# GabrieleCocco/CLFaceDetection

Hardware: NVIDIA B200
Metric: frames_per_sec_1080p (higher is better)
Workload: dtype f64

## Files before the change

clfacedetection_b200/csrc/clfd_pack.h:

```cpp
#pragma once
#include "clfd_internal.h"

namespace clfd {

struct PackedCascade {
    DenseParams dense[2];
    int dense_stumps = 0;
    std::vector<TailStump> tail[2];
    std::vector<DenseStage> stage_tab[2];
    int patch_cut = 0;
    DenseParams patch;
    std::vector<TailStump> patch_tail;
    std::vector<DeepStage> deep_stages;
    std::vector<DeepNode> deep_nodes;
    std::vector<int> tree_first_node;
    std::vector<float> alpha;
};

void pack_cascade(const HostCascade &c, PackedCascade &out);
void pack_sc_level(const HostCascade &c, double factor, int pitch, ScLevel &L, ScNode *out);
bool pack_sc_dense(const HostCascade &c, double scale, DenseParams &P, std::vector<TailStump> &tail,
                   std::vector<DenseStage> &stage_tab);
const char *get_error();

int dense_tile_stride(int win_w, int ystep);
int dense_tile_half(int win_w, int ystep);
int dense_tile_rows(int win_h, int ystep, int tile_h);
int dense_tile_cols(int win_w, int ystep);

}
```

clfacedetection_b200/csrc/haar_pack.cpp:

```cpp
#include <algorithm>
#include <cfloat>
#include <cmath>
#include <cstdarg>
#include <cstdio>
#include <cstdlib>
#include <cstring>

#include "clfd_pack.h"

namespace clfd {

static thread_local char g_error[1024] = "";

void set_error(const char *fmt, ...) {
    va_list ap;
    va_start(ap, fmt);
    vsnprintf(g_error, sizeof g_error, fmt, ap);
    va_end(ap);
}
const char *get_error() { return g_error; }

#define FMT_FAIL(...) do { set_error(__VA_ARGS__); return CLFD_ERR_FORMAT; } while (0)

int build_hidden(HostCascade &c) {
// ... 302 lines not shown
                const int n = c.tr_first_node[t] + j;
                const HostNode &nd = c.nodes[n];
                any3 |= c.hid_nrects[n] == 3;
                for (int k = 0; k < c.hid_nrects[n]; k++) {
                    int dx[4], dy[4];
                    corner_coords(nd, k, dx, dy);
                    for (int q = 0; q < 4; q++) ts.off[k * 4 + q] = tile_offset(dy[q], dx[q]) + (nd.tilted ? (uint32_t)tilt_base : 0u);
                    ts.w[k] = c.hid_weight[(size_t)n * 3 + k];
                }
                ts.thr = nd.threshold;
                ts.a0 = nd.left <= 0 ? c.alpha[a + (-nd.left)] : 0.f;
                ts.a1 = nd.right <= 0 ? c.alpha[a + (-nd.right)] : 0.f;
                ts.meta = (uint32_t)j | ((nd.left > 0 ? (uint32_t)nd.left : kNodeLeaf) << 8) |
                          ((nd.right > 0 ? (uint32_t)nd.right : kNodeLeaf) << 16);
                amax = fmax(amax, fmax(fabs((double)ts.a0), fabs((double)ts.a1)));
            }
            abs_sum += amax;
        }
        ds.first = 0; ds.count = (uint16_t)(c.st_ntrees[i] * P.npt);
        ds.thr = c.hid_thr[i];
        ds.flags = ((!c.is_tree && c.is_stump_based && c.two_rects[i]) ? 1u : 0u) | (any3 ? 2u : 0u) |
                   (c.order_free[i] ? 4u : 0u);
        const double er = (double)(c.st_ntrees[i] * P.npt) * ldexp(1.0, -23) * abs_sum;
        ds.sum_eps = std::isfinite(er) ? (float)(er * 1.0000002) + FLT_MIN : INFINITY;
        ds.sum_eps += 1.0001e-5f * std::fabs(ds.thr);
        if (walk_tree) {
            const uint32_t pass = c.st_child[i] >= 0 ? (uint32_t)pos[c.st_child[i]] : kRouteAccept;
            int p = i;
            while (p >= 0 && c.st_next[p] < 0) p = c.st_parent[p];
            const uint32_t fail = p >= 0 ? (uint32_t)pos[c.st_next[p]] : kRouteReject;
            ds.flags |= ((uint32_t)i << 8) | (pass << 16) | (fail << 24);
            stage_tab[e] = ds;
        }
        if (e < elig) P.stage[e] = ds;
    }
    const bool share_corners = !getenv("CLFD_NO_SHARED_CORNERS");
    int ns = 0, nstump = 0;
    while (ns < elig && nstump + c.st_ntrees[ns] * P.npt <= kMaxDenseStumps) {
        P.stage[ns].first = (uint16_t)nstump;
        std::vector<DenseStump> six, rest;
        for (int t = c.st_first_tree[ns] * P.npt; t < c.st_first_tree[ns + 1] * P.npt; t++) {
            DenseStump st = tail[t];
            bool shared = false;
            if (share_corners && P.npt == 1 && c.hid_nrects[c.tr_first_node[t]] == 2) {
                const uint32_t *A = st.off, *B = st.off + 4;
                static const int pairs[4][2] = {{0, 2}, {3, 1}, {0, 1}, {3, 2}};
                for (const auto &pr : pairs) {
                    const int pl = pr[0], mi = pr[1];
                    if (A[pl] != B[pl] || A[mi] != B[mi]) continue;
                    const int opl = pl == 0 ? 3 : 0, omi = mi == 1 ? 2 : 1;
                    const uint32_t o[6] = {A[pl], A[mi], A[opl], A[omi], B[opl], B[omi]};
                    for (int q = 0; q < 12; q++) st.off[q] = q < 6 ? o[q] : 0;
                    shared = true;
                    break;
                }
            }
            (shared ? six : rest).push_back(st);
        }
        P.stage[ns].n_shared = (uint32_t)six.size();
        for (const auto &st : six) P.stump[nstump++] = st;
        for (const auto &st : rest) P.stump[nstump++] = st;
        ns++;
    }
    P.n_stages = ns;
    {
        static_assert(sizeof(TailStump) == 80, "five 16-byte chunks per record");
        struct Chunk { uint32_t v[4]; };
        std::vector<TailStump> blocked;
        const Chunk *src = reinterpret_cast<const Chunk *>(tail.data());
        int at = 0;
        for (int e = 0; e < E; e++) {
            const int count = c.st_ntrees[order[e]] * P.npt;
            const size_t first = blocked.size();
            blocked.resize(first + (size_t)((count + 31) / 32) * 32);
            Chunk *blk = reinterpret_cast<Chunk *>(blocked.data() + first);
            for (int j = 0; j < count; j++)
                for (int q = 0; q < 5; q++) blk[(size_t)(j >> 5) * 160 + q * 32 + (j & 31)] = src[(size_t)(at + j) * 5 + q];
            if (e < elig) P.stage[e].tail_first = (uint32_t)first;
            if (walk_tree) stage_tab[e].tail_first = (uint32_t)first;
            at += count;
        }
        tail.swap(blocked);
    }
    P.pool_min = 0;
    if (const char *e = getenv("CLFD_POOL_MIN")) P.pool_min = std::max(0, atoi(e));
    P.track_abs = 0;
    for (float v : c.alpha)
        if (std::fabs(v) > 64.f) P.track_abs = 1;
    if (getenv("CLFD_NO_TRACK_ABS")) P.track_abs = 0;
    int nf = 3;
    if (const char *e = getenv("CLFD_N_FIXED")) nf = atoi(e);
    P.n_fixed = nf < 0 ? 0 : (nf > ns ? ns : nf);
}

void pack_cascade(const HostCascade &c, PackedCascade &out) {
    const int S = c.n_stages(), T = c.n_trees(), N = c.n_nodes();
    out.deep_stages.resize(S);
    out.deep_nodes.resize(N);
    out.tree_first_node = c.tr_first_node;
    out.alpha = c.alpha;
    for (int i = 0; i < S; i++) {
        DeepStage &s = out.deep_stages[i];
        memset(&s, 0, sizeof s);
        s.first_tree = c.st_first_tree[i];
        s.ntrees = c.st_ntrees[i];
        s.thr = c.hid_thr[i];
        bool stumps = true;
        for (int t = s.first_tree; t < s.first_tree + s.ntrees; t++) stumps &= c.tr_nnodes[t] == 1;
        const bool dbl = !c.is_tree && c.is_stump_based && c.two_rects[i];
        s.flags = (dbl ? 1 : 0) | (c.order_free[i] ? 2 : 0) | (stumps ? 4 : 0);
        s.parent = c.st_parent[i]; s.next = c.st_next[i]; s.child = c.st_child[i];
    }
    for (int n = 0; n < N; n++) {
        DeepNode &d = out.deep_nodes[n];
        memset(&d, 0, sizeof d);
        const HostNode &nd = c.nodes[n];
        for (int k = 0; k < c.hid_nrects[n]; k++) {
            int dx[4], dy[4];
            corner_coords(nd, k, dx, dy);
            for (int q = 0; q < 4; q++) { d.dx[k * 4 + q] = (uint8_t)dx[q]; d.dy[k * 4 + q] = (uint8_t)dy[q]; }
            d.w[k] = c.hid_weight[(size_t)n * 3 + k];
        }
        d.thr = nd.threshold;
        d.left = nd.left; d.right = nd.right;
        d.flags = (nd.tilted ? 1 : 0) | (c.hid_nrects[n] << 8);
    }

    for (int yi = 0; yi < 2; yi++) pack_dense_one(c, yi + 1, out.dense[yi], out.tail[yi], out.stage_tab[yi], out.dense_stumps);
    out.patch_cut = 0;
    const DenseParams &D = out.dense[0];
    const bool finishes = D.tail_stages == S && D.exec_stages == S && out.dense[1].tail_stages == S;
    if (finishes && !c.has_tilted && !c.is_tree && c.is_stump_based && D.npt == 1 && !D.track_abs && !out.dense[1].track_abs && S >= 8) {
        int cut = 0;
        if (const char *e = getenv("CLFD_PATCH_CUT")) cut = atoi(e);
        if (cut > 0 && cut < S) {
            cut = std::max(cut, std::max(D.n_fixed, out.dense[1].n_fixed));
            std::vector<DenseStage> no_tab;
            int n_stumps = 0;
            pack_dense_one(c, 1, out.patch, out.patch_tail, no_tab, n_stumps, (c.win_w + 1) | 1);
            if (out.patch.tail_stages == S && cut < S) {
                out.patch_cut = cut;
                for (int yi = 0; yi < 2; yi++) out.dense[yi].cut_stages = cut;
            }
        }
    }
}

bool pack_sc_dense(const HostCascade &c, double scale, DenseParams &P, std::vector<TailStump> &tail,
                   std::vector<DenseStage> &stage_tab) {
    HostCascade s = c;
    const int ex = cv_round_d(scale), ey = ex;
    const int ew = cv_round_d((c.win_w - 2) * scale), eh = cv_round_d((c.win_h - 2) * scale);
    const double weight_scale = 1. / (ew * eh);
    int ext_w = std::max(cv_round_d(c.win_w * scale), ex + ew), ext_h = std::max(cv_round_d(c.win_h * scale), ey + eh);
    for (int n = 0; n < c.n_nodes(); n++) {
        const HostNode &nd = c.nodes[n];
        HostNode &d = s.nodes[n];
        const int nr = c.hid_nrects[n];
        double sum0 = 0, area0 = 0;
        const double correction_ratio = weight_scale * (!nd.tilted ? 1 : 0.5);
        for (int k = 0; k < nr; k++) {
            d.rect[k][0] = cv_round_d(nd.rect[k][0] * scale); d.rect[k][2] = cv_round_d(nd.rect[k][2] * scale);
            d.rect[k][1] = cv_round_d(nd.rect[k][1] * scale); d.rect[k][3] = cv_round_d(nd.rect[k][3] * scale);
            int dx[4], dy[4];
            corner_coords(d, k, dx, dy);
            for (int q = 0; q < 4; q++) {
                if (dx[q] < 0 || dy[q] < 0) return false;
                ext_w = std::max(ext_w, dx[q]); ext_h = std::max(ext_h, dy[q]);
            }
            float &w = s.hid_weight[(size_t)n * 3 + k];
            w = (float)(nd.weight[k] * correction_ratio);
            if (k == 0) area0 = d.rect[k][2] * d.rect[k][3];
            else sum0 += w * d.rect[k][2] * d.rect[k][3];
// ... 13 lines not shown
```

clfacedetection_b200/csrc/kernels_clod.cu:

```cuda
#include <algorithm>
#include <cstdint>

#include "clfd_pack.h"
#include "kernels.h"

namespace clfd {

typedef unsigned long long ull;

__device__ __forceinline__ uint32_t smem_u32(const void *p) { return (uint32_t)__cvta_generic_to_shared(p); }

__device__ __forceinline__ void mbar_init(uint64_t *bar, uint32_t count) {
    asm volatile("mbarrier.init.shared::cta.b64 [%0], %1;" ::"r"(smem_u32(bar)), "r"(count));
    asm volatile("fence.mbarrier_init.release.cluster;" ::: "memory");
}
__device__ __forceinline__ void mbar_expect_tx(uint64_t *bar, uint32_t bytes) {
    asm volatile("mbarrier.arrive.expect_tx.shared::cta.b64 _, [%0], %1;" ::"r"(smem_u32(bar)), "r"(bytes) : "memory");
}
__device__ __forceinline__ void mbar_wait(uint64_t *bar, uint32_t parity) {
    asm volatile(
        "{\n"
        ".reg .pred P1;\n"
        "LAB_WAIT:\n"
        "mbarrier.try_wait.parity.shared::cta.b64 P1, [%0], %1;\n"
        "@P1 bra DONE;\n"
        "bra LAB_WAIT;\n"
        "DONE:\n"
        "}" ::"r"(smem_u32(bar)), "r"(parity) : "memory");
}
__device__ __forceinline__ void tma_bulk_g2s(void *dst_smem, const void *src_gmem, uint32_t bytes, uint64_t *bar) {
    asm volatile("cp.async.bulk.shared::cluster.global.mbarrier::complete_tx::bytes [%0], [%1], %2, [%3];"
                 ::"r"(smem_u32(dst_smem)), "l"(src_gmem), "r"(bytes), "r"(smem_u32(bar)) : "memory");
}

__device__ __forceinline__ double window_sigma(int s4, ull q4, double inv_area) {
    const double mean = __dmul_rn((double)s4, inv_area);
    const double v = __dsub_rn(__dmul_rn((double)q4, inv_area), __dmul_rn(mean, mean));
    return v >= 0. ? sqrt(v) : 1.;
}

__device__ __forceinline__ ull sq_rect(const ull *sq, bool sq32, size_t at, int g0, int g1, int g2, int g3) {
    if (sq32) {
        const uint32_t *q = reinterpret_cast<const uint32_t *>(sq) + at;
        return (ull)(uint32_t)(__ldg(q + g0) - __ldg(q + g1) - __ldg(q + g2) + __ldg(q + g3));
    }
    const ull *q = sq + at;
    return __ldg(q + g0) - __ldg(q + g1) - __ldg(q + g2) + __ldg(q + g3);
}

__device__ __forceinline__ void emit_rect(const CascadeArgs &a, const CasLevel &CL, int frame, int px, int py) {
    if (!a.rects) return;
    const ull slot = atomicAdd(a.counters + 0, 1ull);
    if (slot < a.rect_cap) {
        DevRect r;
        r.x = __double2int_rn(__dmul_rn((double)px, CL.factor));
        r.y = __double2int_rn(__dmul_rn((double)py, CL.factor));
        r.w = CL.win_w; r.h = CL.win_h; r.frame = a.frame_base + frame; r.cascade = a.cascade_index;
        a.rects[slot] = r;
    } else {
        atomicAdd(a.counters + 2, 1ull);
    }
}

__device__ __forceinline__ int lds32(uint32_t addr) {
    int v;
    asm volatile("ld.shared.s32 %0, [%1];" : "=r"(v) : "r"(addr));
    return v;
}
template <int IMM>
__device__ __forceinline__ int lds32i(uint32_t addr) {
    int v;
    asm volatile("ld.shared.s32 %0, [%1+%2];" : "=r"(v) : "r"(addr), "n"(IMM));
    return v;
}

#ifdef CLFD_POOLED_STAGES
constexpr bool kPooledStages = true;
#else
constexpr bool kPooledStages = false;
#endif
struct DenseSmemPlan {
    size_t tile, sgf, list, pool, ctl, bar, act, tgt, total;
};
constexpr int kCtlCount = 0, kCtlCountB = 32, kCtlCountC = 64, kCtlInts = 96;
__host__ __device__ inline DenseSmemPlan dense_smem_plan(const DenseParams &P) {
    DenseSmemPlan p;
    const size_t rows = (size_t)(P.tile_h - 1) * P.ystep + P.win_h + 1, windows = (size_t)kTileW * P.tile_h;
    p.tile = 0;
    p.sgf = (rows * P.tile_stride * 4 + 127) & ~(size_t)127;
    if (P.tilted_tile) p.sgf *= 2;
    p.list = p.sgf + windows * sizeof(float);
    p.pool = p.list + windows * sizeof(uint16_t);
    p.ctl = p.pool + (P.pool_min > 0 ? windows * sizeof(uint16_t) : 0);
    p.bar = p.ctl + kCtlInts * sizeof(int);
    p.act = p.tgt = p.total = p.bar + 16;
    if (P.exec_stages > P.tail_stages) {
        p.tgt = p.act + windows * sizeof(uint16_t);
        p.total = p.tgt + windows;
    }
    return p;
}
#ifdef CLFD_TILES_COUNT_TU
constexpr bool kTilesCount = true;
#else
constexpr bool kTilesCount = false;
size_t dense_smem_bytes(const DenseParams &P) { return dense_smem_plan(P).total; }
#endif

struct DenseCtx {
    uint32_t tile;
    const ull *gsq;
    size_t sq_at;
    bool sq32;
    int16_t *codes;
    int sq_pitch;
    int row_mul;
    int ystep, S, half;
    int tx, wy_tile, nx;
    int code_mul;
};

__device__ __forceinline__ uint32_t dense_base(const DenseCtx &c, int wid) {
    return c.tile + (uint32_t)((wid / kTileW) * c.row_mul + (wid & (kTileW - 1)) * 4);
}
__device__ __forceinline__ uint32_t dense_tile_off(const DenseCtx &c, int y, int x) {
    return 4u * (uint32_t)(c.ystep == 1 ? y * c.S + x : y * c.S + (x & 1) * c.half + (x >> 1));
}
__device__ __forceinline__ void dense_write_code(const DenseCtx &c, int wid, int code) {
    const int wx = wid & (kTileW - 1), wy = wid / kTileW;
    c.codes[(size_t)(c.wy_tile + wy) * c.nx + c.tx * kTileW + wx] = (int16_t)code;
}

__device__ __forceinline__ double dense_sigma(const DenseParams &P, const DenseCtx &c, int wid) {
    const int wx = wid & (kTileW - 1), wy = wid / kTileW;
    const int ex = P.eq_x, ey = P.eq_y, eq_w = P.eq_w, eq_h = P.eq_h;
    const uint32_t base = dense_base(c, wid);
    const int s4 = lds32(base + dense_tile_off(c, ey, ex)) - lds32(base + dense_tile_off(c, ey, ex + eq_w)) -
                   lds32(base + dense_tile_off(c, ey + eq_h, ex)) + lds32(base + dense_tile_off(c, ey + eq_h, ex + eq_w));
    const int g0 = ey * c.sq_pitch + ex, g1 = g0 + eq_w, g2 = (ey + eq_h) * c.sq_pitch + ex, g3 = g2 + eq_w;
    const ull q4 = sq_rect(c.gsq, c.sq32, c.sq_at + (size_t)(wy * c.ystep) * c.sq_pitch + wx * c.ystep, g0, g1, g2, g3);
    return window_sigma(s4, q4, P.inv_area);
}
__device__ __forceinline__ double dense_sigma_flat(const DenseParams &P, const DenseCtx &c, int wid, bool &eq_flat) {
    const int wx = wid & (kTileW - 1), wy = wid / kTileW;
    const int ex = P.eq_x, ey = P.eq_y, eq_w = P.eq_w, eq_h = P.eq_h;
    const uint32_t base = dense_base(c, wid);
    const int s4 = lds32(base + dense_tile_off(c, ey, ex)) - lds32(base + dense_tile_off(c, ey, ex + eq_w)) -
                   lds32(base + dense_tile_off(c, ey + eq_h, ex)) + lds32(base + dense_tile_off(c, ey + eq_h, ex + eq_w));
    const int g0 = ey * c.sq_pitch + ex, g1 = g0 + eq_w, g2 = (ey + eq_h) * c.sq_pitch + ex, g3 = g2 + eq_w;
    const ull q4 = sq_rect(c.gsq, c.sq32, c.sq_at + (size_t)(wy * c.ystep) * c.sq_pitch + wx * c.ystep, g0, g1, g2, g3);
    eq_flat = q4 * (ull)(eq_w * eq_h) == (ull)((long long)s4 * s4);
    return window_sigma(s4, q4, P.inv_area);
}

constexpr int kNotFlat = -0x8000;
static __device__ __noinline__ int flat_window_code(const DenseParams &P, const DenseCtx &c, int wid) {
    const uint32_t base = dense_base(c, wid);
    const int W = P.win_w, H = P.win_h;
    const uint32_t S4 = (uint32_t)(lds32(base + dense_tile_off(c, 0, 0)) - lds32(base + dense_tile_off(c, 0, W)) -
                                   lds32(base + dense_tile_off(c, H, 0)) + lds32(base + dense_tile_off(c, H, W)));
    const ull Q4 = sq_rect(c.gsq, c.sq32, c.sq_at + (size_t)((wid / kTileW) * c.ystep) * c.sq_pitch + (wid & (kTileW - 1)) * c.ystep,
                           0, W, H * c.sq_pitch, H * c.sq_pitch + W);
    const uint32_t A = (uint32_t)(W * H);
    if (Q4 * (ull)A != (ull)S4 * (ull)S4) return kNotFlat;
    return (int)__ldg(P.flat_code + S4 / A);
}

struct StumpRegs {
    uint32_t o[12];
    float w0, w1, w2, thr, a0, a1;
    uint32_t meta;
};
__device__ __forceinline__ StumpRegs stump_from_param(const DenseStump &q) {
    StumpRegs r;
#pragma unroll
    for (int i = 0; i < 12; i++) r.o[i] = q.off[i];
    r.w0 = q.w[0]; r.w1 = q.w[1]; r.w2 = q.w[2]; r.thr = q.thr; r.a0 = q.a0; r.a1 = q.a1; r.meta = q.meta;
    return r;
}
__device__ __forceinline__ StumpRegs stump_from_global(const uint4 *__restrict__ rec, int j, bool any3) {
    rec += (j >> 5) * 160 + (j & 31);
    const uint4 q0 = __ldg(rec), q1 = __ldg(rec + 32), q3 = __ldg(rec + 96), q4 = __ldg(rec + 128);
    uint4 q2 = make_uint4(0u, 0u, 0u, 0u);
    if (any3) q2 = __ldg(rec + 64);
    StumpRegs r;
    r.o[0] = q0.x; r.o[1] = q0.y; r.o[2] = q0.z; r.o[3] = q0.w;
    r.o[4] = q1.x; r.o[5] = q1.y; r.o[6] = q1.z; r.o[7] = q1.w;
    r.o[8] = q2.x; r.o[9] = q2.y; r.o[10] = q2.z; r.o[11] = q2.w;
    r.w0 = __uint_as_float(q3.x); r.w1 = __uint_as_float(q3.y); r.w2 = __uint_as_float(q3.z); r.thr = __uint_as_float(q3.w);
// ... 79 lines not shown
    const float d = __fmaf_rn(-q.thr, sg[KK], s32);
    if (NODES) {
        const bool on = at[KK] == (q.meta & 255u);
        near[KK] = near[KK] || (on && fabsf(d) <= m);
        S[KK] = __fadd_rn(S[KK], on ? (d >= 0.f ? q.a1 : q.a0) : 0.f);
        at[KK] = on ? ((d >= 0.f ? q.meta >> 16 : q.meta >> 8) & 255u) : at[KK];
    } else {
        near[KK] = near[KK] || (fabsf(d) <= m);
        const float sel = d >= 0.f ? q.a1 : q.a0;
        S[KK] = __fadd_rn(S[KK], sel);
        if (TRACK) Sa[KK] = __fadd_rn(Sa[KK], fabsf(sel));
    }
}

template <int K, bool FIXED, int ROWSTEP, bool SHARED, bool NODES, bool TRACK>
__device__ __forceinline__ void stump_filter(const StumpRegs &q, bool dbl, bool any3, float eps, const uint32_t (&base)[K],
                                             const float (&sg)[K], float (&S)[K], bool (&near)[K], uint32_t (&at)[K], float (&Sa)[K]) {
    static_assert(K >= 1 && K <= 4, "1..4 windows per thread");
    const bool three = !SHARED && any3 && q.o[11] != 0u;
    uint32_t c[12];
    if (FIXED) {
#pragma unroll
        for (int i = 0; i < (SHARED ? 6 : 12); i++) c[i] = base[0] + q.o[i];
    }
    if (NODES && (q.meta & 255u) == 0u) {
#pragma unroll
        for (int k = 0; k < K; k++) at[k] = 0u;
    }
    stump_filter_window<0, K, FIXED, ROWSTEP, SHARED, NODES, TRACK>(q, dbl, three, eps, c, base, sg, S, near, at, Sa);
    if (K > 1) stump_filter_window<(K > 1 ? 1 : 0), K, FIXED, ROWSTEP, SHARED, NODES, TRACK>(q, dbl, three, eps, c, base, sg, S, near, at, Sa);
    if (K > 2) stump_filter_window<(K > 2 ? 2 : 0), K, FIXED, ROWSTEP, SHARED, NODES, TRACK>(q, dbl, three, eps, c, base, sg, S, near, at, Sa);
    if (K > 3) stump_filter_window<(K > 3 ? 3 : 0), K, FIXED, ROWSTEP, SHARED, NODES, TRACK>(q, dbl, three, eps, c, base, sg, S, near, at, Sa);
}

template <int K, bool FIXED, int ROWSTEP, bool NODES, bool TRACK>
__device__ __forceinline__ void stage_filter(const DenseParams &P, const DenseStage &st, bool resident, int grp, int G,
                                             const uint32_t (&base)[K], const float (&sg)[K], float (&S)[K], bool (&near)[K],
                                             float (&Sa)[K]) {
    uint32_t at[K];
#pragma unroll
    for (int k = 0; k < K; k++) at[k] = 0u;
    const int count = st.count;
    const uint32_t flags = st.flags;
    const bool dbl = flags & 1u, any3 = flags & 2u;
    const float eps = P.filter_eps;
    if (resident && G == 1) {
        const int first = st.first, n6 = (int)st.n_shared;
#pragma unroll 1
        for (int j = 0; j < n6; j++) stump_filter<K, FIXED, ROWSTEP, true, false, TRACK>(stump_from_param(P.stump[first + j]), dbl, false, eps, base, sg, S, near, at, Sa);
#pragma unroll 1
        for (int j = n6; j < count; j++) stump_filter<K, FIXED, ROWSTEP, false, NODES, TRACK>(stump_from_param(P.stump[first + j]), dbl, any3, eps, base, sg, S, near, at, Sa);
    } else {
        const uint4 *__restrict__ rec = reinterpret_cast<const uint4 *>(P.tail + st.tail_first);
        if (NODES) {
            const int npt = P.npt;
#pragma unroll 1
            for (int j = grp * npt; j < count; j += G * npt)
#pragma unroll 1
                for (int i = 0; i < npt; i++)
                    stump_filter<K, FIXED, ROWSTEP, false, true, TRACK>(stump_from_global(rec, j + i, any3), dbl, any3, eps, base, sg, S, near, at, Sa);
        } else {
#pragma unroll 1
            for (int j = grp; j < count; j += G) stump_filter<K, FIXED, ROWSTEP, false, false, TRACK>(stump_from_global(rec, j, any3), dbl, any3, eps, base, sg, S, near, at, Sa);
        }
    }
}

template <bool NODES, bool COUNT, bool TRACK>
__device__ __forceinline__ bool stage_verdict(const DenseParams &P, const DenseCtx &c, const DenseStage &st, float sthr, float seps,
                                              int wid, float S, bool near, float Sa) {
    if (TRACK && !P.force_exact)
        seps = __fadd_ru(__fmul_ru(__fmul_ru((float)st.count, 1.1920930e-7f), Sa), __fadd_ru(__fmul_ru(1.0001e-5f, fabsf(sthr)), 1.2e-38f));
    if (near || !(fabsf(__fadd_rn(S, -sthr)) > seps)) {
        const int r = dense_stage_exact<NODES>(P, c, st.tail_first, st.count, st.flags & 1u, st.thr, wid);
        if (COUNT) {
            atomicAdd(&s_dense_exact, 1u);
            if (r & 2) atomicAdd(&s_dense_near, 1u);
        }
        return r & 1;
    }
    return S >= sthr;
}

template <int ROWSTEP_T, bool TREE, bool NODES, int TILE_H, bool COUNT, bool TRACK>
__device__ __forceinline__ void cascade_tiles_body(const DenseParams &P, const CascadeArgs &a, const int tile0, unsigned char *smem_raw) {
    const DenseSmemPlan plan = dense_smem_plan(P);
    unsigned char *tile = smem_raw + plan.tile;
    float *sgf = reinterpret_cast<float *>(smem_raw + plan.sgf);
    uint16_t *list = reinterpret_cast<uint16_t *>(smem_raw + plan.list);
    int *ctl = reinterpret_cast<int *>(smem_raw + plan.ctl);
    uint64_t *bar = reinterpret_cast<uint64_t *>(smem_raw + plan.bar);

    const int tid = threadIdx.x, lane = tid & 31, warp = tid >> 5;
    const int frame = blockIdx.y;
    const int tile_id = tile0 + blockIdx.x;

    int cl = 0;
    {
        int lo = 0, hi = a.n_cas_levels - 1;
        while (lo < hi) {
            const int mid = (lo + hi + 1) >> 1;
            if (__ldg(&a.cas_levels[mid].tile_base) <= tile_id) lo = mid; else hi = mid - 1;
        }
        cl = lo;
    }
    const CasLevel CL = a.cas_levels[cl];
    const PyrLevel L = a.levels[CL.pyr_level];
    const int local = tile_id - CL.tile_base;
    const int tx = local % CL.tiles_x, ty = local / CL.tiles_x;
    const int ystep = P.ystep;
    constexpr int kTileWindows = kTileW * TILE_H, kDenseSlots = kTileWindows / kDenseThreads;
    constexpr int kDenseChunk = kDenseSlots % 4 == 0 ? 4 : 3;
    static_assert(kDenseSlots % kDenseChunk == 0 && kDenseSlots <= 8, "tile height: 12, 16, 24 or 32 window rows");
    const int px0 = tx * kTileW * ystep, py0 = ty * TILE_H * ystep;
    const int n_wx = min(kTileW, CL.nx - tx * kTileW), n_wy = min(TILE_H, CL.ny - ty * TILE_H);
    const int rows = min((TILE_H - 1) * ystep + P.win_h + 1, L.h + 1 - py0);
    const int cols = ((kTileW - 1) * ystep + P.win_w + 1 + 3) & ~3;
    const int S = P.tile_stride;

    const size_t frame_off = (size_t)frame * a.sum_frame_stride + L.sum_off;
    const int32_t *__restrict__ gsum = a.sum + frame_off + (size_t)py0 * L.sum_pitch + px0;

    for (int i = tid; i < kCtlInts; i += kDenseThreads) ctl[i] = 0;
    if (tid == 0) s_dense_exact = s_dense_near = s_dense_done = 0u;
#ifdef CLFD_TILE_TIMING
    const long long t_start = clock64();
    if (tid == 0) s_dense_t_busy = s_dense_t_p1 = 0u;
#endif
    const int n_tiles_smem = P.tilted_tile ? 2 : 1;
    const size_t tile2_off = ((size_t)((TILE_H - 1) * ystep + P.win_h + 1) * S * 4 + 127) & ~(size_t)127;
    const int32_t *__restrict__ gtil = a.tilted ? a.tilted + frame_off + (size_t)py0 * L.sum_pitch + px0 : gsum;
    if (ystep == 1) {
        if (tid == 0) mbar_init(bar, 1);
        __syncthreads();
        if (tid == 0) mbar_expect_tx(bar, (uint32_t)(rows * cols * 4 * n_tiles_smem));
        for (int r = tid; r < rows * n_tiles_smem; r += kDenseThreads) {
            const int t2 = r >= rows, rr = t2 ? r - rows : r;
            tma_bulk_g2s(tile + (t2 ? tile2_off : 0) + (size_t)rr * S * 4, (t2 ? gtil : gsum) + (size_t)rr * L.sum_pitch,
                         (uint32_t)(cols * 4), bar);
        }
        mbar_wait(bar, 0);
    } else {
        const bool di = a.sum_di != 0;
        const int half = P.tile_half;
        if (di) {
            if (tid == 0) mbar_init(bar, 1);
            __syncthreads();
            const uint32_t hb = (uint32_t)half * 4u;
            if (tid == 0) mbar_expect_tx(bar, (uint32_t)rows * 2u * hb);
            const int32_t *__restrict__ gdi = a.sum + frame_off + (size_t)py0 * L.sum_pitch + (px0 >> 1);
            for (int r = tid; r < rows * 2; r += kDenseThreads) {
                const int odd = r >= rows, rr = odd ? r - rows : r;
                tma_bulk_g2s(tile + (size_t)rr * S * 4 + (odd ? hb : 0u), gdi + (size_t)rr * L.sum_pitch + (odd ? (L.sum_pitch >> 1) : 0), hb, bar);
            }
        }
        const int c4 = cols >> 2, total = rows * c4;
        for (int i = (di ? total : 0) + tid; i < total * n_tiles_smem; i += kDenseThreads) {
            const int t2 = i >= total, ii = t2 ? i - total : i;
            const int r = ii / c4, cq = ii - r * c4;
            const int4 v = __ldg(reinterpret_cast<const int4 *>((t2 ? gtil : gsum) + (size_t)r * L.sum_pitch) + cq);
            int *row = reinterpret_cast<int *>(tile + (t2 ? tile2_off : 0)) + r * S;
            *reinterpret_cast<int2 *>(row + 2 * cq) = make_int2(v.x, v.z);
            *reinterpret_cast<int2 *>(row + half + 2 * cq) = make_int2(v.y, v.w);
        }
        __syncthreads();
        if (di) mbar_wait(bar, 0);
    }

    DenseCtx c;
    c.tile = smem_u32(tile); c.gsq = a.sq; c.sq_at = frame_off + (size_t)py0 * L.sum_pitch + px0; c.sq32 = a.sq32 != 0;
    c.codes = a.codes ? a.codes + (size_t)frame * a.windows_per_frame + CL.win_base : nullptr;
    c.sq_pitch = L.sum_pitch;
    c.row_mul = ystep * S * 4;
    c.ystep = ystep; c.S = S; c.half = P.tile_half;
    c.tx = tx; c.wy_tile = ty * TILE_H; c.nx = CL.nx;
    c.code_mul = P.is_tree ? 2 : 1;
    const float inf = __int_as_float(0x7f800000);

    constexpr int kRowsPerSlot = kDenseThreads / kTileW;
    const int wx = tid & (kTileW - 1), wy0 = tid / kTileW;
    uint32_t alive = 0;
#pragma unroll
    for (int k = 0; k < kDenseSlots; k++) {
        const int wy = wy0 + k * kRowsPerSlot;
        const int wid = wy * kTileW + wx;
        if (wx < n_wx && wy < n_wy) {
            bool eq_flat, live = true;
            sgf[wid] = (float)dense_sigma_flat(P, c, wid, eq_flat);
            if (!COUNT && eq_flat && P.flat_code) {
                const int code = flat_window_code(P, c, wid);
                if (code != kNotFlat) {
                    live = false;
                    if (P.is_tree ? (code & 1) : (code == P.total_stages)) emit_rect(a, CL, frame, px0 + wx * ystep, py0 + wy * ystep);
                }
            }
            if (live) alive |= 1u << k;
        } else {
            sgf[wid] = 1.0f;
        }
    }
    int s = 0;
    for (; s < P.n_fixed; s++) {
        const float sthr = P.stage[s].thr, seps = P.force_exact ? inf : P.stage[s].sum_eps;
#pragma unroll 1
        for (int k0 = 0; k0 < kDenseSlots; k0 += kDenseChunk) {
            const uint32_t m4 = (alive >> k0) & ((1u << kDenseChunk) - 1u);
            if (!__any_sync(0xffffffffu, m4 != 0)) continue;
            uint32_t base[kDenseChunk];
            float sg[kDenseChunk];
            float Ssum[kDenseChunk];
            bool near[kDenseChunk];
#pragma unroll
            for (int k = 0; k < kDenseChunk; k++) {
                const int wy = wy0 + (k0 + k) * kRowsPerSlot;
                base[k] = c.tile + (uint32_t)(wy * c.row_mul + wx * 4);
                sg[k] = sgf[wy * kTileW + wx];
                Ssum[k] = 0.f;
                near[k] = false;
            }
            float Sabs[kDenseChunk];
#pragma unroll
            for (int k = 0; k < kDenseChunk; k++) Sabs[k] = 0.f;
            if (ROWSTEP_T) stage_filter<kDenseChunk, true, ROWSTEP_T, NODES, TRACK>(P, P.stage[s], true, 0, 1, base, sg, Ssum, near, Sabs);
            else stage_filter<kDenseChunk, false, 0, NODES, TRACK>(P, P.stage[s], true, 0, 1, base, sg, Ssum, near, Sabs);
#pragma unroll
            for (int k = 0; k < kDenseChunk; k++) {
                if (!((m4 >> k) & 1u)) continue;
                const int wid = (wy0 + (k0 + k) * kRowsPerSlot) * kTileW + wx;
                if (!stage_verdict<NODES, COUNT, TRACK>(P, c, P.stage[s], sthr, seps, wid, Ssum[k], near[k], Sabs[k])) {
                    alive &= ~(1u << (k0 + k));
                    if (c.codes) dense_write_code(c, wid, s * c.code_mul);
                }
            }
        }
    }

    constexpr int kClassCap = kTileWindows / 32;
    constexpr int kSeg = kTileWindows / kDenseWarps;
    int n_alive;
    uint16_t *cur;
    if (kPooledStages && P.pool_min > 0) {
        uint16_t *cl_in = list, *cl_out = reinterpret_cast<uint16_t *>(smem_raw + plan.pool);
        int *cnt_in = ctl + kCtlCount, *cnt_out = ctl + kCtlCountB, *cnt_zero = ctl + kCtlCountC;
        {
            const int na = __popc(alive);
            if (na) {
                const int cq = (wx + 8 * wy0) & 31;
                int at = atomicAdd(cnt_in + cq, na);
    #pragma unroll
                for (int k = 0; k < kDenseSlots; k++)
                    if ((alive >> k) & 1u) cl_in[cq * kClassCap + at++] = (uint16_t)((wy0 + k * kRowsPerSlot) * kTileW + wx);
            }
        }
        __syncthreads();
            for (;; s++) {
            const int h = cnt_in[lane];
            int incl = h, hmax = h;
    #pragma unroll
            for (int d = 1; d < 32; d <<= 1) {
                const int v = __shfl_up_sync(0xffffffffu, incl, d);
                if (lane >= d) incl += v;
                hmax = max(hmax, __shfl_xor_sync(0xffffffffu, hmax, d));
            }
            const int excl = incl - h, tot = __shfl_sync(0xffffffffu, incl, 31);
            if (tot == 0) return;
            n_alive = tot;
            if (!(P.pool_min > 0 && tot > P.pool_min && s < P.tail_stages)) {
                for (int r = warp; r < h; r += kDenseWarps) {
                    const int i = excl + r;
                    const int w = i % kDenseWarps, p = i / kDenseWarps;
                    const int nw = (tot - w + kDenseWarps - 1) / kDenseWarps, Rw = (nw + 31) >> 5;
                    const int col = p / Rw, row = p - col * Rw;
                    cl_out[w * kSeg + row * 32 + col] = cl_in[lane * kClassCap + r];
                }
                __syncthreads();
                break;
            }
            int R = (tot + 31) >> 5;
            {
                int best = 0x7fffffff;
                for (int r = R; r <= hmax; r++) {
                    int e = max(h - r, 0);
    #pragma unroll
                    for (int d = 16; d > 0; d >>= 1) e += __shfl_xor_sync(0xffffffffu, e, d);
                    const int cost = r * 9 + 5 * min(r, e);
                    if (cost < best) { best = cost; R = r; }
                }
            }
            const int q = (R + kDenseWarps - 1) / kDenseWarps;
            const int r_begin = warp * q, r_end = min(R, r_begin + q);
            if (tid < 32) cnt_zero[tid] = 0;
            const float sthr = P.stage[s].thr, seps = P.force_exact ? inf : P.stage[s].sum_eps;
            auto fetch = [&](int r, bool &valid) -> int {
                const int i = r + lane * R;
                valid = i < tot;
                int cc = 0;
    #pragma unroll
                for (int step = 16; step > 0; step >>= 1) {
                    const int e_t = __shfl_sync(0xffffffffu, excl, (cc + step) & 31);
                    if (e_t <= i) cc += step;
                }
                const int e_c = __shfl_sync(0xffffffffu, excl, cc);
                return valid ? (int)cl_in[cc * kClassCap + (i - e_c)] : 0;
            };
            auto keep_pool = [&](bool valid, int wid, float Ssum, bool near, float Sabs) {
                const bool pass = valid && stage_verdict<NODES, COUNT, TRACK>(P, c, P.stage[s], sthr, seps, wid, Ssum, near, Sabs);
                if (pass) {
                    const int cq = (wid + 8 * (wid / kTileW)) & 31;
                    cl_out[cq * kClassCap + atomicAdd(cnt_out + cq, 1)] = (uint16_t)wid;
                }
                if (valid && !pass && c.codes) dense_write_code(c, wid, s * c.code_mul);
            };
            for (int r = r_begin; r < r_end; r += 2) {
                bool v0, v1 = false;
                const int wid0 = fetch(r, v0);
                if (r + 1 < r_end) {
                    const int wid1 = fetch(r + 1, v1);
                    const uint32_t base[2] = {dense_base(c, wid0), dense_base(c, wid1)};
                    const float sg[2] = {sgf[wid0], sgf[wid1]};
                    float Ssum[2] = {0.f, 0.f};
                    bool near[2] = {false, false};
                    float Sabs[2] = {0.f, 0.f};
                    stage_filter<2, false, 0, NODES, TRACK>(P, P.stage[s], s < P.n_stages, 0, 1, base, sg, Ssum, near, Sabs);
                    keep_pool(v0, wid0, Ssum[0], near[0], Sabs[0]);
                    keep_pool(v1, wid1, Ssum[1], near[1], Sabs[1]);
                } else {
                    const uint32_t base[1] = {dense_base(c, wid0)};
                    const float sg[1] = {sgf[wid0]};
                    float Ssum[1] = {0.f};
                    bool near[1] = {false};
                    float Sabs[1] = {0.f};
                    stage_filter<1, false, 0, NODES, TRACK>(P, P.stage[s], s < P.n_stages, 0, 1, base, sg, Ssum, near, Sabs);
                    keep_pool(v0, wid0, Ssum[0], near[0], Sabs[0]);
                }
            }
            __syncthreads();
            uint16_t *tl = cl_in; cl_in = cl_out; cl_out = tl;
            int *tc = cnt_in; cnt_in = cnt_out; cnt_out = cnt_zero; cnt_zero = tc;
        }

        cur = cl_out + warp * kSeg;
    } else {
        const int na = __popc(alive), cq = (wx + 8 * wy0) & 31;
        int at = na ? atomicAdd(ctl + kCtlCount + cq, na) : 0;
        __syncthreads();
        const int h = ctl[kCtlCount + lane];
        int incl = h;
#pragma unroll
        for (int d = 1; d < 32; d <<= 1) {
            const int v = __shfl_up_sync(0xffffffffu, incl, d);
            if (lane >= d) incl += v;
        }
        n_alive = __shfl_sync(0xffffffffu, incl, 31);
        if (n_alive == 0) return;
        at += __shfl_sync(0xffffffffu, incl - h, cq);
#pragma unroll
        for (int k = 0; k < kDenseSlots; k++) {
            if ((alive >> k) & 1u) {
                const int i = at++;
                const int w = i % kDenseWarps, p = i / kDenseWarps;
                const int nw = (n_alive - w + kDenseWarps - 1) / kDenseWarps, Rw = (nw + 31) >> 5;
                const int col = p / Rw, row = p - col * Rw;
                list[w * kSeg + row * 32 + col] = (uint16_t)((wy0 + k * kRowsPerSlot) * kTileW + wx);
            }
        }
        __syncthreads();
        cur = list + warp * kSeg;
    }

#ifdef CLFD_TILE_TIMING
    if (lane == 0) atomicAdd(&s_dense_t_p1, (unsigned int)(clock64() - t_start));
#endif
    int n = (n_alive - warp + kDenseWarps - 1) / kDenseWarps;
    bool dealt = true;
    for (; s < P.cut_stages && n > 0; s++) {
        const float sthr = P.stage[s].thr, seps = P.force_exact ? inf : P.stage[s].sum_eps;
        int n_next = 0;
        auto keep = [&](bool valid, int wid, float Ssum, bool near, float Sabs) {
            const bool pass = valid && stage_verdict<NODES, COUNT, TRACK>(P, c, P.stage[s], sthr, seps, wid, Ssum, near, Sabs);
            const unsigned m = __ballot_sync(0xffffffffu, pass);
            if (pass) cur[n_next + __popc(m & ((1u << lane) - 1u))] = (uint16_t)wid;
            n_next += __popc(m);
            if (valid && !pass && c.codes) dense_write_code(c, wid, s * c.code_mul);
        };
        if (n > P.g1_min) {
            const int R = (n + 31) >> 5;
            for (int r = 0; r < R; r += 2) {
                const int c0 = dealt ? (n - r + R - 1) / R : min(32, n - 32 * r);
                if (r + 1 < R) {
                    const int c1 = dealt ? (n - r - 1 + R - 1) / R : min(32, n - 32 * (r + 1));
                    const bool v0 = lane < c0, v1 = lane < c1;
                    const int wid0 = cur[32 * r + (v0 ? lane : 0)], wid1 = cur[32 * r + 32 + (v1 ? lane : 0)];
                    __syncwarp();
                    const uint32_t base[2] = {dense_base(c, wid0), dense_base(c, wid1)};
                    const float sg[2] = {sgf[wid0], sgf[wid1]};
                    float Ssum[2] = {0.f, 0.f};
                    bool near[2] = {false, false};
                    float Sabs[2] = {0.f, 0.f};
                    stage_filter<2, false, 0, NODES, TRACK>(P, P.stage[s], s < P.n_stages, 0, 1, base, sg, Ssum, near, Sabs);
                    keep(v0, wid0, Ssum[0], near[0], Sabs[0]);
                    keep(v1, wid1, Ssum[1], near[1], Sabs[1]);
                } else {
                    const bool v0 = lane < c0;
                    const int wid0 = cur[32 * r + (v0 ? lane : 0)];
                    __syncwarp();
                    const uint32_t base[1] = {dense_base(c, wid0)};
                    const float sg[1] = {sgf[wid0]};
                    float Ssum[1] = {0.f};
                    bool near[1] = {false};
                    float Sabs[1] = {0.f};
                    stage_filter<1, false, 0, NODES, TRACK>(P, P.stage[s], s < P.n_stages, 0, 1, base, sg, Ssum, near, Sabs);
                    keep(v0, wid0, Ssum[0], near[0], Sabs[0]);
                }
            }
        } else {
            int lw = 4;
            while (lw > 0 && (1 << (lw - 1)) >= n) lw--;
            const int slot = lane & ((1 << lw) - 1), grp = lane >> lw, G = 32 >> lw;
            const bool valid = slot < n;
            const int wid0 = cur[valid ? slot : 0];
            __syncwarp();
            const uint32_t base[1] = {dense_base(c, wid0)};
            const float sg[1] = {sgf[wid0]};
            float Ssum[1] = {0.f};
            bool near[1] = {false};
            float Sabs[1] = {0.f};
            if (valid) stage_filter<1, false, 0, NODES, TRACK>(P, P.stage[s], s < P.n_stages, grp, G, base, sg, Ssum, near, Sabs);
            float acc = Ssum[0], acc_abs = Sabs[0];
            unsigned nr = near[0];
            for (int d = 1 << lw; d < 32; d <<= 1) {
                acc = __fadd_rn(acc, __shfl_xor_sync(0xffffffffu, acc, d));
                if (TRACK) acc_abs = __fadd_rn(acc_abs, __shfl_xor_sync(0xffffffffu, acc_abs, d));
                nr |= __shfl_xor_sync(0xffffffffu, nr, d);
            }
            keep(lane < n, wid0, acc, nr != 0, acc_abs);
        }
        __syncwarp();
        n = n_next;
        dealt = false;
    }
    if (TREE) {
        if (n == 0) return;
        uint16_t *act = reinterpret_cast<uint16_t *>(smem_raw + plan.act) + warp * kSeg;
        unsigned char *tgt = smem_raw + plan.tgt;
        const int e0 = s;
        for (int e = e0; e < P.exec_stages && n > 0; e++) {
            int n_wait = 0, n_act = 0;
            const int R = (n + 31) >> 5;
            for (int r = 0; r < R; r++) {
                const int c0 = dealt ? (n - r + R - 1) / R : min(32, n - 32 * r);
                const bool v = lane < c0;
// ... 658 lines not shown
```

Baseline: 2856.

## Enable pooled cross-warp stage evaluation with dynamic row claiming by default

Turns the previously compile-time-disabled pooled stage path into a default runtime path for stump cascades when it does not reduce CTAs per SM. Surviving windows are pooled across the whole CTA, and warps claim row pairs dynamically through a shared atomic counter. This replaces static per-warp segments so early stages stay load-balanced as windows die out. It also simplifies the row-count choice to a heuristic and lowers the default fixed-stage count when pooling is on. The cost is extra shared memory, additional __syncthreads and atomics per stage.

```diff
diff --git a/clfacedetection_b200/csrc/clfd_pack.h b/clfacedetection_b200/csrc/clfd_pack.h
--- a/clfacedetection_b200/csrc/clfd_pack.h
+++ b/clfacedetection_b200/csrc/clfd_pack.h
@@ -27,5 +27,6 @@
 int dense_tile_half(int win_w, int ystep);
 int dense_tile_rows(int win_h, int ystep, int tile_h);
 int dense_tile_cols(int win_w, int ystep);
+bool dense_pooled(const DenseParams &P);
 
 }
diff --git a/clfacedetection_b200/csrc/haar_pack.cpp b/clfacedetection_b200/csrc/haar_pack.cpp
--- a/clfacedetection_b200/csrc/haar_pack.cpp
+++ b/clfacedetection_b200/csrc/haar_pack.cpp
@@ -408,13 +408,15 @@
         }
         tail.swap(blocked);
     }
-    P.pool_min = 0;
+    constexpr int kPoolMin = 256;
+    P.pool_min = !c.is_tree && P.npt == 1 && patch_stride == 0 ? kPoolMin : 0;
     if (const char *e = getenv("CLFD_POOL_MIN")) P.pool_min = std::max(0, atoi(e));
+    if (!dense_pooled(P)) P.pool_min = 0;
     P.track_abs = 0;
     for (float v : c.alpha)
         if (std::fabs(v) > 64.f) P.track_abs = 1;
     if (getenv("CLFD_NO_TRACK_ABS")) P.track_abs = 0;
-    int nf = 3;
+    int nf = P.pool_min > 0 ? 2 : 3;
     if (const char *e = getenv("CLFD_N_FIXED")) nf = atoi(e);
     P.n_fixed = nf < 0 ? 0 : (nf > ns ? ns : nf);
 }
diff --git a/clfacedetection_b200/csrc/kernels_clod.cu b/clfacedetection_b200/csrc/kernels_clod.cu
--- a/clfacedetection_b200/csrc/kernels_clod.cu
+++ b/clfacedetection_b200/csrc/kernels_clod.cu
@@ -74,27 +74,32 @@
     return v;
 }
 
-#ifdef CLFD_POOLED_STAGES
-constexpr bool kPooledStages = true;
-#else
-constexpr bool kPooledStages = false;
-#endif
 struct DenseSmemPlan {
     size_t tile, sgf, list, pool, ctl, bar, act, tgt, total;
+    bool pooled;
 };
-constexpr int kCtlCount = 0, kCtlCountB = 32, kCtlCountC = 64, kCtlInts = 96;
+constexpr int kCtlClaim = 64, kCtlInts = 96;
+constexpr size_t kSmemPerSm = 228 * 1024, kSmemPerCta = 1024 + 64;
+constexpr int kDenseCtasPerSm = 4;
+__host__ __device__ inline int dense_ctas_per_sm(size_t bytes) {
+    const int n = (int)(kSmemPerSm / (bytes + kSmemPerCta));
+    return n < kDenseCtasPerSm ? n : kDenseCtasPerSm;
+}
 __host__ __device__ inline DenseSmemPlan dense_smem_plan(const DenseParams &P) {
     DenseSmemPlan p;
     const size_t rows = (size_t)(P.tile_h - 1) * P.ystep + P.win_h + 1, windows = (size_t)kTileW * P.tile_h;
+    const size_t act = P.exec_stages > P.tail_stages ? windows * sizeof(uint16_t) + windows : 0;
     p.tile = 0;
     p.sgf = (rows * P.tile_stride * 4 + 127) & ~(size_t)127;
     if (P.tilted_tile) p.sgf *= 2;
     p.list = p.sgf + windows * sizeof(float);
     p.pool = p.list + windows * sizeof(uint16_t);
-    p.ctl = p.pool + (P.pool_min > 0 ? windows * sizeof(uint16_t) : 0);
+    const size_t fixed = p.pool + kCtlInts * sizeof(int) + 16 + act;
+    p.pooled = P.pool_min > 0 && dense_ctas_per_sm(fixed + windows * sizeof(uint16_t)) == dense_ctas_per_sm(fixed);
+    p.ctl = p.pool + (p.pooled ? windows * sizeof(uint16_t) : 0);
     p.bar = p.ctl + kCtlInts * sizeof(int);
     p.act = p.tgt = p.total = p.bar + 16;
-    if (P.exec_stages > P.tail_stages) {
+    if (act) {
         p.tgt = p.act + windows * sizeof(uint16_t);
         p.total = p.tgt + windows;
     }
@@ -105,6 +110,7 @@
 #else
 constexpr bool kTilesCount = false;
 size_t dense_smem_bytes(const DenseParams &P) { return dense_smem_plan(P).total; }
+bool dense_pooled(const DenseParams &P) { return dense_smem_plan(P).pooled; }
 #endif
 
 struct DenseCtx {
@@ -350,6 +356,24 @@
     return S >= sthr;
 }
 
+__device__ __forceinline__ void class_prefix(int h, int &excl, int &tot, int &hmax) {
+    const int lane = threadIdx.x & 31;
+    int incl = h;
+    hmax = h;
+#pragma unroll
+    for (int d = 1; d < 32; d <<= 1) {
+        const int v = __shfl_up_sync(0xffffffffu, incl, d);
+        if (lane >= d) incl += v;
+        hmax = max(hmax, __shfl_xor_sync(0xffffffffu, hmax, d));
+    }
+    excl = incl - h;
+    tot = __shfl_sync(0xffffffffu, incl, 31);
+}
+__device__ __forceinline__ int pooled_rows(int n, int hmax) {
+    const int r0 = (n + 31) >> 5;
+    return min(hmax, r0 + ((r0 + 3) >> 2));
+}
+
 template <int ROWSTEP_T, bool TREE, bool NODES, int TILE_H, bool COUNT, bool TRACK>
 __device__ __forceinline__ void cascade_tiles_body(const DenseParams &P, const CascadeArgs &a, const int tile0, unsigned char *smem_raw) {
     const DenseSmemPlan plan = dense_smem_plan(P);
@@ -505,93 +529,56 @@
 
     constexpr int kClassCap = kTileWindows / 32;
     constexpr int kSeg = kTileWindows / kDenseWarps;
-    int n_alive;
-    uint16_t *cur;
-    if (kPooledStages && P.pool_min > 0) {
-        uint16_t *cl_in = list, *cl_out = reinterpret_cast<uint16_t *>(smem_raw + plan.pool);
-        int *cnt_in = ctl + kCtlCount, *cnt_out = ctl + kCtlCountB, *cnt_zero = ctl + kCtlCountC;
-        {
-            const int na = __popc(alive);
-            if (na) {
-                const int cq = (wx + 8 * wy0) & 31;
-                int at = atomicAdd(cnt_in + cq, na);
-    #pragma unroll
-                for (int k = 0; k < kDenseSlots; k++)
-                    if ((alive >> k) & 1u) cl_in[cq * kClassCap + at++] = (uint16_t)((wy0 + k * kRowsPerSlot) * kTileW + wx);
+    const int na = __popc(alive), cq = (wx + 8 * wy0) & 31;
+    int *const cnt0 = ctl + 32 * ((s & 1) ^ 1);
+    int at = na ? atomicAdd(cnt0 + cq, na) : 0;
+    __syncthreads();
+    int h = cnt0[lane], excl, n_alive, hmax;
+    class_prefix(h, excl, n_alive, hmax);
+    if (n_alive == 0) return;
+    at += __shfl_sync(0xffffffffu, excl, cq);
+    if (plan.pooled && n_alive > P.pool_min && s < P.cut_stages) {
+        uint16_t *const cls = list + kTileWindows;
+        int R = pooled_rows(n_alive, hmax);
+#pragma unroll
+        for (int k = 0; k < kDenseSlots; k++) {
+            if ((alive >> k) & 1u) {
+                const int i = at++;
+                list[(i % R) * 32 + i / R] = (uint16_t)((wy0 + k * kRowsPerSlot) * kTileW + wx);
             }
         }
         __syncthreads();
-            for (;; s++) {
-            const int h = cnt_in[lane];
-            int incl = h, hmax = h;
-    #pragma unroll
-            for (int d = 1; d < 32; d <<= 1) {
-                const int v = __shfl_up_sync(0xffffffffu, incl, d);
-                if (lane >= d) incl += v;
-                hmax = max(hmax, __shfl_xor_sync(0xffffffffu, hmax, d));
-            }
-            const int excl = incl - h, tot = __shfl_sync(0xffffffffu, incl, 31);
-            if (tot == 0) return;
-            n_alive = tot;
-            if (!(P.pool_min > 0 && tot > P.pool_min && s < P.tail_stages)) {
-                for (int r = warp; r < h; r += kDenseWarps) {
-                    const int i = excl + r;
-                    const int w = i % kDenseWarps, p = i / kDenseWarps;
-                    const int nw = (tot - w + kDenseWarps - 1) / kDenseWarps, Rw = (nw + 31) >> 5;
-                    const int col = p / Rw, row = p - col * Rw;
-                    cl_out[w * kSeg + row * 32 + col] = cl_in[lane * kClassCap + r];
-                }
-                __syncthreads();
-                break;
-            }
-            int R = (tot + 31) >> 5;
-            {
-                int best = 0x7fffffff;
-                for (int r = R; r <= hmax; r++) {
-                    int e = max(h - r, 0);
-    #pragma unroll
-                    for (int d = 16; d > 0; d >>= 1) e += __shfl_xor_sync(0xffffffffu, e, d);
-                    const int cost = r * 9 + 5 * min(r, e);
-                    if (cost < best) { best = cost; R = r; }
-                }
-            }
-            const int q = (R + kDenseWarps - 1) / kDenseWarps;
-            const int r_begin = warp * q, r_end = min(R, r_begin + q);
-            if (tid < 32) cnt_zero[tid] = 0;
+        for (;;) {
+            int *const cnt = ctl + 32 * (s & 1);
+            if (tid < 32) ctl[32 * ((s & 1) ^ 1) + tid] = 0;
+            const int lim = n_alive - lane * R;
             const float sthr = P.stage[s].thr, seps = P.force_exact ? inf : P.stage[s].sum_eps;
-            auto fetch = [&](int r, bool &valid) -> int {
-                const int i = r + lane * R;
-                valid = i < tot;
-                int cc = 0;
-    #pragma unroll
-                for (int step = 16; step > 0; step >>= 1) {
-                    const int e_t = __shfl_sync(0xffffffffu, excl, (cc + step) & 31);
-                    if (e_t <= i) cc += step;
-                }
-                const int e_c = __shfl_sync(0xffffffffu, excl, cc);
-                return valid ? (int)cl_in[cc * kClassCap + (i - e_c)] : 0;
-            };
-            auto keep_pool = [&](bool valid, int wid, float Ssum, bool near, float Sabs) {
+            auto keep = [&](bool valid, int wid, float Ssum, bool near, float Sabs) {
                 const bool pass = valid && stage_verdict<NODES, COUNT, TRACK>(P, c, P.stage[s], sthr, seps, wid, Ssum, near, Sabs);
                 if (pass) {
-                    const int cq = (wid + 8 * (wid / kTileW)) & 31;
-                    cl_out[cq * kClassCap + atomicAdd(cnt_out + cq, 1)] = (uint16_t)wid;
+                    const int k = (wid + 8 * (wid / kTileW)) & 31;
+                    cls[k * kClassCap + atomicAdd(cnt + k, 1)] = (uint16_t)wid;
                 }
                 if (valid && !pass && c.codes) dense_write_code(c, wid, s * c.code_mul);
             };
-            for (int r = r_begin; r < r_end; r += 2) {
-                bool v0, v1 = false;
-                const int wid0 = fetch(r, v0);
-                if (r + 1 < r_end) {
-                    const int wid1 = fetch(r + 1, v1);
+            for (;;) {
+                int r = 0;
+                if (lane == 0) r = 2 * atomicAdd(ctl + kCtlClaim, 1);
+                r = __shfl_sync(0xffffffffu, r, 0);
+                if (r >= R) break;
+                const bool v0 = r < lim;
+                const int wid0 = list[32 * r + (v0 ? lane : 0)];
+                if (r + 1 < R) {
+                    const bool v1 = r + 1 < lim;
+                    const int wid1 = list[32 * r + 32 + (v1 ? lane : 0)];
                     const uint32_t base[2] = {dense_base(c, wid0), dense_base(c, wid1)};
                     const float sg[2] = {sgf[wid0], sgf[wid1]};
                     float Ssum[2] = {0.f, 0.f};
                     bool near[2] = {false, false};
                     float Sabs[2] = {0.f, 0.f};
                     stage_filter<2, false, 0, NODES, TRACK>(P, P.stage[s], s < P.n_stages, 0, 1, base, sg, Ssum, near, Sabs);
-                    keep_pool(v0, wid0, Ssum[0], near[0], Sabs[0]);
-                    keep_pool(v1, wid1, Ssum[1], near[1], Sabs[1]);
+                    keep(v0, wid0, Ssum[0], near[0], Sabs[0]);
+                    keep(v1, wid1, Ssum[1], near[1], Sabs[1]);
                 } else {
                     const uint32_t base[1] = {dense_base(c, wid0)};
                     const float sg[1] = {sgf[wid0]};
@@ -599,29 +586,34 @@
                     bool near[1] = {false};
                     float Sabs[1] = {0.f};
                     stage_filter<1, false, 0, NODES, TRACK>(P, P.stage[s], s < P.n_stages, 0, 1, base, sg, Ssum, near, Sabs);
-                    keep_pool(v0, wid0, Ssum[0], near[0], Sabs[0]);
+                    keep(v0, wid0, Ssum[0], near[0], Sabs[0]);
                 }
             }
             __syncthreads();
-            uint16_t *tl = cl_in; cl_in = cl_out; cl_out = tl;
-            int *tc = cnt_in; cnt_in = cnt_out; cnt_out = cnt_zero; cnt_zero = tc;
-        }
-
-        cur = cl_out + warp * kSeg;
+            s++;
+            h = cnt[lane];
+            class_prefix(h, excl, n_alive, hmax);
+            if (n_alive == 0) return;
+            if (!(n_alive > P.pool_min && s < P.cut_stages)) {
+                for (int j = warp; j < h; j += kDenseWarps) {
+                    const int i = excl + j;
+                    const int w = i % kDenseWarps, p = i / kDenseWarps;
+                    const int nw = (n_alive - w + kDenseWarps - 1) / kDenseWarps, Rw = (nw + 31) >> 5;
+                    const int col = p / Rw, row = p - col * Rw;
+                    list[w * kSeg + row * 32 + col] = cls[lane * kClassCap + j];
+                }
+                __syncthreads();
+                break;
+            }
+            R = pooled_rows(n_alive, hmax);
+            for (int j = warp; j < h; j += kDenseWarps) {
+                const int i = excl + j;
+                list[(i % R) * 32 + i / R] = cls[lane * kClassCap + j];
+            }
+            if (tid == 0) ctl[kCtlClaim] = 0;
+            __syncthreads();
+        }
     } else {
-        const int na = __popc(alive), cq = (wx + 8 * wy0) & 31;
-        int at = na ? atomicAdd(ctl + kCtlCount + cq, na) : 0;
-        __syncthreads();
-        const int h = ctl[kCtlCount + lane];
-        int incl = h;
-#pragma unroll
-        for (int d = 1; d < 32; d <<= 1) {
-            const int v = __shfl_up_sync(0xffffffffu, incl, d);
-            if (lane >= d) incl += v;
-        }
-        n_alive = __shfl_sync(0xffffffffu, incl, 31);
-        if (n_alive == 0) return;
-        at += __shfl_sync(0xffffffffu, incl - h, cq);
 #pragma unroll
         for (int k = 0; k < kDenseSlots; k++) {
             if ((alive >> k) & 1u) {
@@ -633,8 +625,8 @@
             }
         }
         __syncthreads();
-        cur = list + warp * kSeg;
-    }
+    }
+    uint16_t *cur = list + warp * kSeg;
 
 #ifdef CLFD_TILE_TIMING
     if (lane == 0) atomicAdd(&s_dense_t_p1, (unsigned int)(clock64() - t_start));
```

Measured after the change: 2972, median of 6. 1.04x the previous value.
